# Vipermaseg/libagmv

Hardware: AMD Instinct MI355X
Metric: frames/s encode+decode (AGMV hot path: quantise+classify+assemble, parse+reconstruct), synthetic (higher is better)
Workload: dtype u8; 1 GPU; c3: 1024-frame 1920x1080 agmv_synth_v1, HIGH_QUALITY palette, OPT_III (512 colours); frames_per_gpu=1024, width=1920, height=1080, palette=512 colours, reference histogram build (GPU histogram + host pick), parallelism=1024 frames per rank, 1 rank(s), no data-path collective

## Files before the change

### libagmv_amd/csrc/agmv_decode_hip.hip

```cpp
#include <hip/hip_runtime.h>

#include <stdint.h>
#include <stdlib.h>
#include <string.h>
#include <type_traits>

#include "agmv_hip_impl.h"

#ifndef DEC_T_OVERRIDE
#define DEC_T_OVERRIDE 256
#endif
constexpr int DEC_T = DEC_T_OVERRIDE;
#ifndef DEC_BPB
#define DEC_BPB 24
#endif
constexpr int DEC_STAGE = DEC_T * DEC_BPB;
constexpr int DEC_SR = DEC_STAGE / 4 / DEC_T;
constexpr int DEC_MAX_SLICES = 32;

struct dec_ws {
	uint32_t* d_dirty;
	size_t dirty_cap;
	bool dep_split;
	uint32_t* d_parse_ws;
	size_t parse_ws_cap;
	uint32_t* d_fp_ws;
	size_t fp_ws_cap;
	uint32_t* d_fp_fstate;
	uint32_t fp_frames;
	uint32_t* d_fstate_call;
	size_t fstate_call_cap;
	uint32_t* d_nent_own;
	size_t nent_cap;
	hipStream_t aux_stream;
	hipEvent_t ev_fork;
	hipEvent_t ev_slice[DEC_MAX_SLICES];
};

static dec_ws* dec_area(agmv_hip_ctx* c) { return (dec_ws*)c->ws[AREA_DEC]; }

static void dec_free(void* p)
{
	dec_ws* d = (dec_ws*)p;
	(void)hipFree(d->d_dirty); (void)hipFree(d->d_parse_ws); (void)hipFree(d->d_fp_ws); (void)hipFree(d->d_nent_own);
	(void)hipFree(d->d_fstate_call);
	if (d->ev_fork) (void)hipEventDestroy(d->ev_fork);
	for (int i = 0; i < DEC_MAX_SLICES; i++) if (d->ev_slice[i]) (void)hipEventDestroy(d->ev_slice[i]);
	if (d->aux_stream) (void)hipStreamDestroy(d->aux_stream);
	free(d);
}

static int need_dec_ctx(agmv_hip_ctx* c, bool palette)
{
	if (agmv_hip_enter(c, palette)) return -1;
	return palette && !agmv_hip_area(c, AREA_DEC, sizeof(dec_ws), dec_free) ? -1 : 0;
}

template <class F>
static void dec_flags(F&& f) { f(); }
template <class F, class... Rest>
static void dec_flags(F&& f, bool flag, Rest... rest) { dec_flags([&](auto... r_) { if (flag) f(std::true_type(), r_...); else f(std::false_type(), r_...); }, rest...); }
#define DEC_LAUNCH(k, grid, block, s, A, ...) do { \
	dec_flags([&](auto... b_) { hipLaunchKernelGGL((k<decltype(b_)::value...>), grid, block, 0, s, A); }, __VA_ARGS__); \
	CK(hipGetLastError()); } while (0)

__device__ __forceinline__ bool is_flag(uint32_t b) { return b == FILL_FLAG || b == NORMAL_FLAG || b == COPY_FLAG; }

struct ByteSrc {
	const uint8_t* p;
	uint32_t cap;
	__device__ __forceinline__ uint32_t operator()(uint32_t pos) const { return pos < cap ? p[pos] : 0u; }
};

struct StagedSrc {
	const __attribute__((address_space(3))) uint8_t* lds;
	uint32_t lo, len;
	const uint8_t* p;
	uint32_t cap;
	__device__ __forceinline__ uint32_t operator()(uint32_t pos) const
	{
		const uint32_t d = pos - lo;
		if (d < len) return lds[d];
		return pos < cap ? p[pos] : 0u;
	}
};

__global__ __launch_bounds__(64) void k_parse_serial(const uint8_t* __restrict__ bits, unsigned long long stride,
                                                     const uint32_t* __restrict__ bpos_a, uint32_t n_frames,
                                                     uint32_t nblk, int mode512, uint32_t* __restrict__ offsets,
                                                     uint32_t* __restrict__ nentered)
// ... 81 lines not shown
struct ParseLds {
	uint8_t b[PC + PHALO];
	unsigned long long esc[PNSEG + 2];
	uint16_t jl[NLV][PC];
};

constexpr int PCD = ((PC + PHALO) / 4 + 63) / 64;

__device__ __forceinline__ void load_chunk(uint32_t (&raw)[PCD], const uint8_t* fbits, uint32_t cap, uint32_t cs, int lane)
{
#pragma unroll
	for (int q = 0; q < PCD; q++) {
		const uint32_t pos = cs + 4u * (uint32_t)(q * 64 + lane);
		raw[q] = (q * 64 + lane < (PC + PHALO) / 4 && pos < cap) ? *(const uint32_t*)(fbits + pos) : 0u;
	}
}

template <bool M512, int NLV>
__device__ __forceinline__ uint32_t parse_chunk_nodes(ParseLds<NLV>& S, uint16_t* rank_at, uint16_t* npos, uint16_t* eo, uint16_t* n0,
                                                      const uint32_t (&raw)[PCD], uint32_t bpos, uint32_t cs, int lane)
{
#pragma unroll
	for (int q = 0; q < PCD; q++) {
		const int i = q * 64 + lane;
		if (i < (PC + PHALO) / 4) ((uint32_t*)S.b)[i] = raw[q];
	}
	wave_lds_sync();
	uint32_t mtot = 0, by[PNSEG];
#pragma unroll
	for (int sg = 0; sg < PNSEG; sg++) by[sg] = S.b[sg * 64 + lane];
#pragma unroll
	for (int sg = 0; sg < PNSEG; sg++) {
		const uint32_t p = sg * 64 + lane;
		const bool node = is_flag(by[sg]) && cs + p <= bpos;
		const unsigned long long m = __ballot(node);
		const uint32_t r = mtot + __builtin_amdgcn_mbcnt_hi((uint32_t)(m >> 32), __builtin_amdgcn_mbcnt_lo((uint32_t)m, 0u));
		rank_at[p] = (uint16_t)r;
		if (node) npos[r] = (uint16_t)p;
		mtot += (uint32_t)__popcll(m);
		if (M512) {
			const unsigned long long em = __ballot((by[sg] & 0x7fu) == 127u);
			if (lane == 0) S.esc[sg] = em;
		}
	}
	if (M512) {
		const unsigned long long em = __ballot((S.b[PC + lane] & 0x7fu) == 127u);
		if (lane == 0) { S.esc[PNSEG] = em; S.esc[PNSEG + 1] = 0; }
	}
	wave_lds_sync();
	const bool more = cs + PC <= bpos;
	for (uint32_t k = lane; k < mtot; k += 64) {
		const uint32_t p = npos[k], byte = S.b[p];
		uint32_t e = p + 1u;
		if (byte == FILL_FLAG) e += M512 ? 1u + ((S.b[p + 1] & 0x7fu) == 127u ? 1u : 0u) : 1u;
		else if (byte == NORMAL_FLAG) {
			if (M512) {
				const uint32_t sg = e >> 6, sh = e & 63u;
				const unsigned long long lo = S.esc[sg], hi = S.esc[sg + 1];
				const uint32_t m = (uint32_t)(sh ? (lo >> sh) | (hi << (64u - sh)) : lo);
				uint32_t pos = 0;
#pragma unroll
				for (int i = 0; i < 16; i++) pos += 1u + ((m >> pos) & 1u);
				e += pos;
			} else e += 16u;
		}
		uint32_t j = J_END, n = 0;
		if (cs + e <= bpos) {
			n = 1;
			if (e >= (uint32_t)PC) j = J_EXIT | (e - PC);
			else {
				const uint32_t nx = rank_at[e];
				j = nx < mtot ? nx : (more ? J_EXIT : J_END);
			}
		}
		S.jl[0][k] = (uint16_t)j;
		if (eo) eo[k] = (uint16_t)(e | n << 15);
		if (n0) n0[k] = (uint16_t)n;
	}
	wave_lds_sync();
	return mtot;
}

template <bool M512>
__global__ __launch_bounds__(64) void k_parse_chunks(ParseArgs A)
{
	__shared__ ParseLds<2> S;
	__shared__ uint16_t nn[2][PC];
	const int lane = threadIdx.x;
	if (A.nbad && *A.nbad == 0) return;
	for (uint32_t f = blockIdx.y; f < A.n_frames; f += gridDim.y) {
	const uint32_t bpos = A.bpos[f], g0 = f * A.cpf, nch = parse_nch(A, f, bpos);
	const uint8_t* fbits = A.bits + (size_t)f * A.stride;
	uint32_t nxt[PCD];
	if (blockIdx.x < nch) load_chunk(nxt, fbits, (uint32_t)A.stride, blockIdx.x * PC, lane);
	for (uint32_t c = blockIdx.x; c < nch; c += gridDim.x) {
		const uint32_t g = g0 + c, cs = c * PC;
		uint32_t raw[PCD];
#pragma unroll
		for (int q = 0; q < PCD; q++) raw[q] = nxt[q];
		if (c + gridDim.x < nch) load_chunk(nxt, fbits, (uint32_t)A.stride, (c + gridDim.x) * PC, lane);
		if (A.vm && lane < PC / 64) A.vm[(size_t)f * A.maxR * FOWN + c * (PC / 64) + lane] = 0ull;
		const uint32_t mtot = parse_chunk_nodes<M512>(S,  nn[1],  S.jl[1], nullptr, nn[0], raw, bpos, cs, lane);
		const uint32_t k0 = lane < 33 ? nn[1][lane] : 0u;
		wave_lds_sync();
#pragma unroll
		for (int lv = 0; lv < PCL; lv++) {
			const uint16_t *js = S.jl[lv & 1], *ns = nn[lv & 1];
			uint16_t *jd = S.jl[(lv + 1) & 1], *nd = nn[(lv + 1) & 1];
			for (uint32_t k = lane; k < mtot; k += 64) {
				uint32_t j = js[k], n = ns[k];
				if (j < J_EXIT) { n += ns[j]; j = js[j]; }
				jd[k] = (uint16_t)j;
				nd[k] = (uint16_t)n;
			}
			wave_lds_sync();
		}
		if (lane < 33) {
			uint32_t ex = X_END, cnt = 0;
			if (cs + lane <= bpos) {
				uint32_t k = k0;
				if (k >= mtot) { if (cs + PC <= bpos) ex = 0; }
				else {
					const uint16_t *jf = S.jl[PCL & 1], *nf = nn[PCL & 1];
					do { cnt += nf[k]; k = jf[k]; } while (k < J_EXIT);
					if (k != J_END) ex = k & 0x3Fu;
				}
			}
			A.summ[(size_t)g * 33 + lane] = (uint16_t)(ex << 10 | cnt);
		}
		wave_lds_sync();
	}
	}
}

constexpr int PSB = 32;
__global__ __launch_bounds__(64) void k_parse_stitch(ParseArgs A)
{
	const int lane = threadIdx.x;
	if (A.nbad && *A.nbad == 0) return;
	for (uint32_t f = blockIdx.x; f < A.n_frames; f += gridDim.x) {
	const uint32_t c0 = f * A.cpf, nch = parse_nch(A, f, A.bpos[f]);
	if (nch == 0) continue;
	const uint16_t* rows = A.summ + (size_t)c0 * 33 + (lane < 33 ? lane : 0);
	uint32_t o = 0, kb = 0;
	uint32_t nxt[PSB];
#pragma unroll
	for (int u = 0; u < PSB; u++) nxt[u] = rows[(size_t)min((uint32_t)u, nch - 1u) * 33];
	for (uint32_t c = 0; c < nch; c += PSB) {
		uint32_t row[PSB];
#pragma unroll
		for (int u = 0; u < PSB; u++) row[u] = nxt[u];
#pragma unroll
		for (int u = 0; u < PSB; u++) nxt[u] = rows[(size_t)min(c + PSB + u, nch - 1u) * 33];
		uint32_t mine = 0;
#pragma unroll
		for (int u = 0; u < PSB; u++) {
			if (lane == u) mine = kb << 8 | o;
			if (c + u < nch && o != 0xFFu) {
				const uint32_t v = __builtin_amdgcn_readlane(row[u], __builtin_amdgcn_readfirstlane(o));
				kb += v & 0x3FFu;
				o = (v >> 10) == X_END ? 0xFFu : v >> 10;
			}
		}
		if (lane < PSB && c + lane < nch) A.centry[c0 + c + lane] = mine;
	}
	if (lane == 0) A.nentered[f] = min(A.nblk, kb + 1u);
	}
}

template <bool M512>
__global__ __launch_bounds__(64) void k_parse_emit(ParseArgs A)
{
	__shared__ ParseLds<PEL + 1> S;
	__shared__ uint16_t eo[PC];
	uint8_t* mark = S.b;
	static_assert(PEL >= 2 && PC + PHALO >= PC, "rank_at / npos borrow jl[PEL-1] / jl[PEL], the marks borrow the bytes");
	const int lane = threadIdx.x;
	if (A.nbad && *A.nbad == 0) return;
	for (uint32_t f = blockIdx.y; f < A.n_frames; f += gridDim.y) {
	const uint32_t bpos = A.bpos[f], g0 = f * A.cpf, nch = parse_nch(A, f, bpos);
	const uint8_t* fbits = A.bits + (size_t)f * A.stride;
	uint32_t* off = A.offsets + (size_t)f * A.nblk;
	uint32_t nxt[PCD], ce_n = 0;
	if (blockIdx.x < nch) { ce_n = A.centry[g0 + blockIdx.x]; load_chunk(nxt, fbits, (uint32_t)A.stride, blockIdx.x * PC, lane); }
	for (uint32_t c = blockIdx.x; c < nch; c += gridDim.x) {
		const uint32_t ce = ce_n, o = ce & 0xFFu, kb = ce >> 8;
		uint32_t raw[PCD];
#pragma unroll
		for (int q = 0; q < PCD; q++) raw[q] = nxt[q];
		if (c + gridDim.x < nch) {
			ce_n = A.centry[g0 + c + gridDim.x];
			load_chunk(nxt, fbits, (uint32_t)A.stride, (c + gridDim.x) * PC, lane);
		}
		unsigned long long* fvm = A.vm ? A.vm + (size_t)f * A.maxR * FOWN : nullptr;
		if (c == 0 && lane == 0) {
			if (fvm) atomicOr(fvm, 1ull); else off[0] = 0;
		}
		if (o == 0xFFu) continue;
		if (kb + 1u >= A.nblk) continue;
		const uint32_t cs = c * PC;
		const uint32_t mtot = parse_chunk_nodes<M512>(S,  S.jl[PEL - 1],  S.jl[PEL], eo, nullptr, raw, bpos, cs, lane);
		const uint32_t k0 = cs + o <= bpos ? S.jl[PEL - 1][o] : mtot;
		for (uint32_t k = lane; k < mtot; k += 64) mark[k] = 0;
		wave_lds_sync();
		if (k0 < mtot) {
#pragma unroll
			for (int lv = 0; lv < PEL; lv++) {
				for (uint32_t k = lane; k < mtot; k += 64) {
					uint32_t j = S.jl[lv][k];
					if (j < J_EXIT) j = S.jl[lv][j];
					S.jl[lv + 1][k] = (uint16_t)j;
				}
				wave_lds_sync();
			}
			if (lane == 0)
				for (uint32_t k = k0; k < J_EXIT; k = S.jl[PEL][k]) mark[k] = 1;
			wave_lds_sync();
#pragma unroll
			for (int lv = PEL - 1; lv >= 0; lv--) {
				for (uint32_t k = lane; k < mtot; k += 64) {
					const uint32_t j = S.jl[lv][k];
					if (mark[k] && j < J_EXIT) mark[j] = 1;
				}
				wave_lds_sync();
			}
			uint32_t base = kb + 1u;
			for (uint32_t kg = 0; kg < mtot; kg += 64) {
				const uint32_t k = kg + lane;
				const uint32_t ev = k < mtot ? eo[k] : 0u;
				const bool on = k < mtot && mark[k] && (ev & 0x8000u);
				const unsigned long long m = __ballot(on);
				const uint32_t kk = base + __builtin_amdgcn_mbcnt_hi((uint32_t)(m >> 32), __builtin_amdgcn_mbcnt_lo((uint32_t)m, 0u));
				if (on && kk < A.nblk) {
					const uint32_t pos = cs + (ev & 0x7FFFu);
					if (fvm) atomicOr(fvm + (pos >> 6), 1ull << (pos & 63u)); else off[kk] = pos;
				}
				base += (uint32_t)__popcll(m);
			}
		}
		wave_lds_sync();
	}
	}
}

constexpr int FROW = FC / 4 + 1;
constexpr uint32_t FX_SLIDE = 64u, FX_END = 65u, FX_UNSET = 66u, FX_MERGE = 128u;
constexpr int FP_REPAIRS = 24;
constexpr int FP_LDS = 64 * FROW + 1;

struct FpArgs {
	const uint8_t* bits;
	unsigned long long stride;
	const uint32_t* bpos;
	uint4* rec;
	unsigned long long* vm;
	uint32_t* kb;
	uint32_t* fstate;
	uint32_t* offsets;
	uint32_t* nentered;
	uint32_t n_frames, nblk, maxR;
	uint32_t* nbad;
	uint32_t* tidx;
	uint32_t tpfd;
	uint32_t* dirty;
	uint32_t ndirty;
};
constexpr uint32_t TIDX_NONE = 0xFFFFFFFFu;

__device__ __forceinline__ __amdgpu_buffer_rsrc_t uniform_rsrc(const void* p, uint32_t bytes)
{
	const uint64_t a = (uint64_t)p;
	const uint32_t lo = (uint32_t)__builtin_amdgcn_readfirstlane((int)(uint32_t)a), hi = (uint32_t)__builtin_amdgcn_readfirstlane((int)(uint32_t)(a >> 32));
	return __builtin_amdgcn_make_buffer_rsrc((void*)((uint64_t)hi << 32 | lo), 0, __builtin_amdgcn_readfirstlane((int)bytes), 0x00020000);
}

__device__ __forceinline__ uint32_t ctz64(unsigned long long m) { return (uint32_t)__builtin_ctzll(m); }
__device__ __forceinline__ unsigned long long above(uint32_t q) { return (~0ull << q) << 1; }

template <bool M512>
__device__ __forceinline__ void fp_walk_region(const FpArgs& A, uint32_t* s_b, uint32_t f, uint32_t r, uint32_t forced, uint32_t bpos, int lane)
{
	const uint8_t* fbits = A.bits + (size_t)f * A.stride;
	const uint32_t cap = (uint32_t)A.stride;
	const long sb = (long)r * FRB - FH * FC;
	uint32_t raw[16];
	{
		const __amdgpu_buffer_rsrc_t rs = uniform_rsrc(fbits, cap & ~3u);
		const uint32_t o0 = (sb < 0 ? 0xFFFFFF00u : (uint32_t)sb) + 4u * (uint32_t)lane;
		const uint32_t o1 = (uint32_t)(sb + FH * FC) + 4u * (uint32_t)lane;
		raw[0] = (uint32_t)__builtin_amdgcn_raw_buffer_load_b32(rs, o0, 0, 0);
#pragma unroll
		for (int k = 1; k < 16; k++) raw[k] = (uint32_t)__builtin_amdgcn_raw_buffer_load_b32(rs, o1 + 256u * (uint32_t)(k - 1), 0, 0);
	}
	{
		uint32_t* row = s_b + (lane >> 4) * FROW + (lane & 15);
#pragma unroll
		for (int k = 0; k < 16; k++) row[k * 4 * FROW] = raw[k];
	}
	wave_lds_sync();
	const long cb = sb + (long)lane * FC;
	unsigned long long F, C, L, E = 0;
	{
		auto zero7 = [](uint32_t v) -> uint32_t { return ~(((v & 0x7F7F7F7Fu) + 0x7F7F7F7Fu) | v) & 0x80808080u; };
		uint32_t f2[2] = {0, 0}, c2[2] = {0, 0}, lc2[2] = {0, 0}, e2[2] = {0, 0};
		auto place = [](uint32_t acc, uint32_t x128, int sh) -> uint32_t { return acc | (sh == 0 ? x128 >> 7 : x128 << (sh - 7)); };
		auto pair128 = [](uint32_t z0, uint32_t z1) -> uint32_t {
			return __builtin_amdgcn_udot4(z1, 0x80402010u, __builtin_amdgcn_udot4(z0, 0x08040201u, 0u, false), false);
		};
#pragma unroll
		for (int j = 0; j < 16; j += 2) {
			const uint32_t w0 = s_b[lane * FROW + j], w1 = s_b[lane * FROW + j + 1];
			const uint32_t zlc0 = zero7((w0 | 0x10101010u) ^ 0x5E5E5E5Eu), zn0 = zero7(w0 ^ 0x2F2F2F2Fu);
			const uint32_t zlc1 = zero7((w1 | 0x10101010u) ^ 0x5E5E5E5Eu), zn1 = zero7(w1 ^ 0x2F2F2F2Fu);
			const int h = j >> 3, sh = 4 * (j & 7);
			lc2[h] = place(lc2[h], pair128(zlc0, zlc1), sh);
			c2[h] = place(c2[h], pair128(zlc0 & (w0 << 3), zlc1 & (w1 << 3)), sh);
			f2[h] = place(f2[h], pair128(zlc0 | zn0, zlc1 | zn1), sh);
			if (M512) e2[h] = place(e2[h], pair128(((w0 & 0x7F7F7F7Fu) + 0x01010101u) & 0x80808080u, ((w1 & 0x7F7F7F7Fu) + 0x01010101u) & 0x80808080u), sh);
		}
		F = (unsigned long long)f2[1] << 32 | f2[0]; C = (unsigned long long)c2[1] << 32 | c2[0];
		L = ((unsigned long long)lc2[1] << 32 | lc2[0]) ^ C; E = (unsigned long long)e2[1] << 32 | e2[0];
	}
	const long lim_l = (long)bpos - cb;
	const int lim = lim_l > 1000 ? 1000 : (lim_l < -1000 ? -1000 : (int)lim_l);
// ... 2 lines not shown
		const long nv = lim_l + 1;
		const unsigned long long ok = nv <= 0 ? 0ull : (nv < 64 ? (1ull << nv) - 1ull : ~0ull);
		F &= ok;
		safe = ok >> 3;
	}
	const bool more = lim >= FC;
	unsigned long long En = 0;
	unsigned long long D;
	{
		unsigned long long L3 = 0;
		if (M512) {
			const uint32_t lo = (uint32_t)__shfl_down((int)(uint32_t)E, 1, 64), hi = (uint32_t)__shfl_down((int)(uint32_t)(E >> 32), 1, 64);
			En = lane < 63 ? ((unsigned long long)hi << 32 | lo) : 0ull;
			L3 = L & ((E >> 1) | (En << 63));
			L &= ~L3;
		}
		D = (F & ~(C | L | L3)) | (F & ((L << 1) | (L3 << 1) | (L3 << 2))) | (F & ~safe);
	}
	const int first = forced != FX_UNSET ? FH : 0;
	const bool walker = lane >= first && lane < 63 && cb >= 0;
	const uint32_t* mine = s_b + lane * FROW;
	const uint32_t behind = mine[FROW];
	unsigned long long V = 0, Q = 0;
	uint32_t xo = FX_UNSET, applied = FX_UNSET;
	uint32_t want = (lane == first && forced != FX_UNSET) ? forced : FX_SLIDE;
	for (int round = 0; round < 66; round++) {
		const bool need = walker && want != applied;
		if (__ballot(need) == 0) break;
		bool go = false;
		uint32_t q = 0, res = xo;
		unsigned long long Vw = 0, Qw = 0;
		if (need) {
			applied = want;
			if (want == FX_END) { V = 0; Q = 0; res = FX_END; }
			else {
				const uint32_t x = want == FX_SLIDE ? 0u : want;
				Vw = want == FX_SLIDE ? 0ull : 1ull << x;
				const unsigned long long m = F >> x;
				if (m == 0) { V = Vw; Q = 0; res = more ? FX_SLIDE : FX_END; }
				else {
					q = x + ctz64(m);
					if ((Q >> q) & 1ull) { V = Vw | (V & above(q)); Q &= ~0ull << q; }
					else go = true;
				}
			}
		}
		uint32_t wres = FX_UNSET;
		for (;;) {
			if (__ballot(go) == 0) break;
			{
				const bool merged = go && ((Q >> q) & 1ull);
				wres = merged ? FX_MERGE + q : wres;
				go = go && !merged;
			}
			const unsigned long long hiq = ~0ull << q;
			const unsigned long long dq = (D & hiq) | (Q & (hiq << 1));
			const uint32_t d = dq ? ctz64(dq) : 64u;
			const bool str = go && d != q;
			if (__ballot(str) != 0) {
				const unsigned long long nodes = F & hiq & (d >= 64u ? ~0ull : ~(~0ull << d));
				const uint32_t last = 63u - (uint32_t)__builtin_clzll(nodes | 1ull);
				const uint32_t e = last + (((C >> last) & 1ull) ? 1u : (((L >> last) & 1ull) ? 2u : 3u));
				Qw |= str ? nodes : 0ull;
				Vw |= str ? ((nodes & C) << 1) | ((nodes & L) << 2) | ((nodes & ~(C | L)) << 3) : 0ull;
				const unsigned long long m = F >> (e & 63u);
				const bool inside = e < 64u && m != 0;
				const uint32_t stop = e >= 64u ? e - 64u : (more ? FX_SLIDE : FX_END);
				wres = (str && !inside) ? stop : wres;
				const uint32_t p = e + ctz64(m | (1ull << 63));
				const bool arrived = str && inside;
				const bool merged = arrived && ((Q >> (p & 63u)) & 1ull);
				wres = merged ? FX_MERGE + p : wres;
				q = arrived ? p : q;
				go = go && (!str || (inside && !merged));
			}
			const bool sing = go && ((D >> q) & 1ull);
			if (__ballot(sing) != 0) {
				const uint32_t d0 = mine[q >> 2], d1 = mine[(q >> 2) + 1];
				const uint32_t two = __builtin_amdgcn_alignbyte((q >> 2) == 15u ? behind : d1, d0, q & 3u);
				const uint32_t t = two & 0xFFu;
				const bool isN = t == NORMAL_FLAG, isC = t == COPY_FLAG;
				uint32_t l1 = isC ? 1u : 2u + ((M512 && ((two >> 8) & 0x7Fu) == 127u) ? 1u : 0u);
				if (__ballot(sing && isN) != 0) {
					uint32_t len = 16;
					if (M512) {
						const uint32_t q1 = q + 1u;
						const uint32_t m = (uint32_t)((q1 < 64u ? E >> q1 : 0ull) | (En << (63u - q)));
						uint32_t pos = 0;
#pragma unroll
						for (int i = 0; i < 16; i++) pos += 1u + ((m >> pos) & 1u);
						len = pos;
					}
					if (isN) l1 = 1u + len;
				}
				const uint32_t e = q + l1;
				const bool over = (int)e > lim;
				const bool cnt = sing && !over;
				Qw |= cnt ? 1ull << q : 0ull;
				Vw |= cnt ? (1ull << q) << l1 : 0ull;
				const unsigned long long m = F >> (e & 63u);
				const bool inside = cnt && e < 64u && m != 0;
				const uint32_t stop = over ? FX_END : (e >= 64u ? e - 64u : (more ? FX_SLIDE : FX_END));
				wres = (sing && !inside) ? stop : wres;
				q = inside ? e + ctz64(m) : q;
				go = go && (!sing || inside);
			}
		}
		if (need && wres != FX_UNSET) {
			if (wres >= FX_MERGE) {
				const uint32_t mq = wres - FX_MERGE;
				V = Vw | (V & above(mq)); Q = Qw | (Q & (~0ull << mq));
			} else { V = Vw; Q = Qw; res = wres; }
		}
		if (need) xo = res;
		const uint32_t px = (uint32_t)__shfl_up((int)xo, 1, 64);
		if (walker && lane > first) want = px;
	}
	const bool own = lane >= FH && lane < 63;
	if (own) A.vm[((size_t)f * A.maxR + r) * FOWN + (lane - FH)] = walker ? V : 0ull;
	const uint32_t n = wave_sum(own && walker ? (uint32_t)__popcll(V) : 0u);
	const uint32_t ein = forced != FX_UNSET ? forced : (uint32_t)__builtin_amdgcn_readlane((int)xo, FH - 1);
	const uint32_t xout = (uint32_t)__builtin_amdgcn_readlane((int)xo, 62);
	if (lane == 0) A.rec[(size_t)f * A.maxR + r] = make_uint4(ein, xout, n, 0u);
	wave_lds_sync();
}

template <bool M512>
__global__ __launch_bounds__(64) __attribute__((amdgpu_waves_per_eu(6, 8))) void k_fp_walk(FpArgs A)
{
	__shared__ uint32_t s_b[FP_LDS];
	const int lane = threadIdx.x;
	if (blockIdx.x == 0 && blockIdx.y == 0 && lane == 0) *A.nbad = 0;
	for (uint32_t f = blockIdx.y; f < A.n_frames; f += gridDim.y) {
		const uint32_t bpos = A.bpos[f];
		const uint32_t nreg = min(bpos / FRB + 1u, A.maxR);
		for (uint32_t r = blockIdx.x; r < nreg; r += gridDim.x)
			fp_walk_region<M512>(A, s_b, f, r, r == 0 ? 0u : FX_UNSET, bpos, lane);
	}
}

template <bool M512>
__global__ __launch_bounds__(64) __attribute__((amdgpu_waves_per_eu(8, 8))) void k_fp_finish(FpArgs A)
{
	__shared__ uint32_t s_b[FP_LDS];
	const uint32_t f = blockIdx.x;
	const int lane = threadIdx.x;
	const uint32_t bpos = A.bpos[f];
	const uint32_t nreg = min(bpos / FRB + 1u, A.maxR);
	uint4* rec = A.rec + (size_t)f * A.maxR;
	if (A.tidx)
		for (uint32_t t = lane; t <= A.tpfd; t += 64) A.tidx[(size_t)f * (A.tpfd + 1) + t] = TIDX_NONE;
	int budget = FP_REPAIRS;
	for (uint32_t start = 1;;) {
		uint32_t bad = 0xFFFFFFFFu;
		for (uint32_t r0 = start & ~63u; r0 < nreg && bad == 0xFFFFFFFFu; r0 += 64) {
			const uint32_t r = r0 + lane;
			const bool in = r < nreg && r >= start;
			const uint32_t x = in ? __hip_atomic_load(&rec[r].x, __ATOMIC_RELAXED, __HIP_MEMORY_SCOPE_AGENT) : 0u;
			const uint32_t yp = in ? __hip_atomic_load(&rec[r - 1].y, __ATOMIC_RELAXED, __HIP_MEMORY_SCOPE_AGENT) : 0u;
			const unsigned long long bm = __ballot(in && x != yp);
			if (bm) bad = r0 + ctz64(bm);
		}
		if (bad == 0xFFFFFFFFu) break;
		if (budget-- == 0) {
			if (lane == 0) { A.fstate[f] = FS_BAD; atomicAdd(A.nbad, 1u); }
			return;
		}
		const uint32_t want = __builtin_amdgcn_readfirstlane(__hip_atomic_load(&rec[bad - 1].y, __ATOMIC_RELAXED, __HIP_MEMORY_SCOPE_AGENT));
		fp_walk_region<M512>(A, s_b, f, bad, want, bpos, lane);
		__builtin_amdgcn_fence(__ATOMIC_RELEASE, "agent");
		__builtin_amdgcn_fence(__ATOMIC_ACQUIRE, "agent");
		start = bad + 1;
	}
	uint32_t run = 0;
	for (uint32_t r0 = 0; r0 < nreg; r0 += 64) {
		const uint32_t r = r0 + lane;
// ... 602 lines not shown
	else {
#pragma unroll
		for (int k = 0; k < 16; k++) cur[k] = 0;
	}
	if (A.prev_iframe) load_block(A.prev_iframe, poff, A.w, icol);
	else {
#pragma unroll
		for (int k = 0; k < 16; k++) icol[k] = 0;
	}
	uint32_t stale = 0xFFFFu, istale = 0xFFFFu;
	bool dep = false;
	for (uint32_t f = 0; f < A.n_frames; f++) {
		bool fill_written = false;
		const uint32_t own3 = cur[3], own3s = (stale >> 3) & 1u;
		if (active && blk < A.nentered[f]) {
			ByteSrc src{A.bits + (size_t)f * A.stride, (uint32_t)A.stride};
			const uint32_t o = BM ? bm_offset_of(A.vm, A.kb, A.maxR, A.bpos[f], f, blk) : A.offsets[(size_t)f * A.nblk + blk];
			decode_block<M512>(src, o, A.bpos[f], s_pal, cur, icol, istale, stale, fill_written);
		}
		const int nbl = nb_lane < 0 ? 0 : nb_lane;
		const uint32_t left = (uint32_t)__builtin_amdgcn_readlane((int)cur[7], nbl);
		const uint32_t lefts = ((uint32_t)__builtin_amdgcn_readlane((int)stale, nbl) >> 7) & 1u;
		if (is_last && fill_written) {
			const uint32_t c = A.bw == 1 ? own3 : left;
#pragma unroll
			for (int k = 0; k < 16; k++) cur[k] = c;
			stale = (A.bw == 1 ? own3s : lefts) ? 0xFFFFu : 0u;
		}
		if (((A.first_fc + f) & 3u) == 0) {
#pragma unroll
			for (int k = 0; k < 16; k++) icol[k] = cur[k];
			istale = stale;
		}
		if (active) store_block(A.out + (size_t)f * npx, poff, A.w, cur);
		if (active && stale) dep = true;
	}
	if (dep) A.dirty[nwords + 1] = 1u;
}

static int check_slab(const uint8_t* d_bits, size_t stride)
{
	if ((stride & 3u) || stride < 4 || ((uintptr_t)d_bits & 3u)) return agmv_hip_err("agmv_hip: bitstream slab and stride must be 4-byte aligned");
	return 0;
}

struct DecRows {
	const uint8_t* bits;
	size_t stride;
	const uint32_t* bpos;
	uint32_t *offsets, *nentered;
	uint32_t n_frames, nblk;
};
static DecRows rows_range(DecRows r, uint32_t f0, uint32_t f1)
{
	r.bits += (size_t)f0 * r.stride; r.bpos += f0; r.nentered += f0; r.n_frames = f1 - f0;
	if (r.offsets) r.offsets += (size_t)f0 * r.nblk;
	return r;
}
struct DecPix {
	uint32_t w, h, first_fc;
	uint32_t* out;
	const uint32_t *prev, *prev_iframe;
};

static uint32_t dirty_words(uint32_t nblk) { return (nblk + 31) / 32 + 2; }

enum ParseMode { PARSE_FAST, PARSE_ROBUST, PARSE_SERIAL };
static ParseMode parse_mode()
{
	const char* m = getenv("AGMV_HIP_PARSE");
	return !m ? PARSE_FAST : strcmp(m, "robust") == 0 ? PARSE_ROBUST : strcmp(m, "serial") == 0 ? PARSE_SERIAL : PARSE_FAST;
}

static uint32_t parse_grid_x(agmv_hip_ctx* c, uint32_t n_frames, size_t cap)
{
	uint32_t gx = (uint32_t)(((size_t)c->n_cu * 512 + n_frames - 1) / n_frames);
	if (gx < 32) gx = 32;
	if (gx > 256) gx = 256;
	if (gx > cap) gx = (uint32_t)cap;
	return gx < 1 ? 1 : gx;
}

static int parse_launch_robust(agmv_hip_ctx* c, const DecRows& r, size_t ws_frames, hipStream_t s,
                               const uint32_t* fstate, const uint32_t* nbad, unsigned long long* vm, uint32_t maxR)
{
	const size_t cpf = (r.stride + PC) / PC, maxchunks = cpf * ws_frames;
	if (maxchunks >> 32) return agmv_hip_err("agmv_hip: parser batch too large (%zu chunk rows)", maxchunks);
	dec_ws* d = dec_area(c);
	CK(agmv_hip_dev_grow(&d->d_parse_ws, &d->parse_ws_cap, (maxchunks + (maxchunks * 33 + 1) / 2 + 16) * 4, 1));
	ParseArgs A;
	memset(&A, 0, sizeof(A));
	A.bits = r.bits; A.stride = r.stride; A.bpos = r.bpos; A.offsets = r.offsets; A.nentered = r.nentered;
	A.cpf = (uint32_t)cpf; A.centry = d->d_parse_ws; A.summ = (uint16_t*)(A.centry + maxchunks);
	A.n_frames = r.n_frames; A.nblk = r.nblk; A.fstate = fstate; A.vm = vm; A.maxR = maxR; A.nbad = nbad;
	const uint32_t n = r.n_frames;
	const dim3 grid(parse_grid_x(c, n, fstate && cpf > 32 ? 32 : cpf), fstate ? (n < 64u ? n : 64u) : (n < 65535u ? n : 65535u));
	const int m512 = c->mode512;
	DEC_LAUNCH(k_parse_chunks, grid, dim3(64), s, A, m512);
	hipLaunchKernelGGL(k_parse_stitch, dim3(fstate ? (n < 1024u ? n : 1024u) : n), dim3(64), 0, s, A);
	CK(hipGetLastError());
	DEC_LAUNCH(k_parse_emit, grid, dim3(64), s, A, m512);
	return 0;
}

static int parse_launch(agmv_hip_ctx* c, const DecRows& r, size_t ws_frames, hipStream_t s, DecArgs* bm, uint32_t* fstate = nullptr)
{
	const bool robust_only = parse_mode() == PARSE_ROBUST;
	const uint32_t n_frames = r.n_frames;
	dec_ws* d = dec_area(c);
	d->d_fp_fstate = nullptr; d->fp_frames = 0;
	if (!bm && (n_frames > 65535u || robust_only)) return parse_launch_robust(c, r, ws_frames, s, nullptr, nullptr, nullptr, 0);
	if (n_frames > 65535u) return agmv_hip_err("agmv_hip: more than 65535 frames in one parser launch");
	const size_t maxR = (r.stride + FRB - 1) / FRB + 1, nreg = maxR * ws_frames;
	const uint32_t tpfd = (r.nblk + DEC_T - 1) / DEC_T;
	const size_t b_rec = nreg * sizeof(uint4), b_vm = nreg * FOWN * 8, b_kb = nreg * 4, b_fs = ((ws_frames * 4 + 15) & ~(size_t)15);
	const size_t b_tx = bm ? (((size_t)ws_frames * (tpfd + 1) * 4 + 15) & ~(size_t)15) : 0;
	CK(agmv_hip_dev_grow(&d->d_fp_ws, &d->fp_ws_cap, b_rec + b_vm + b_kb + b_fs + b_tx + 16, 1));
	FpArgs A;
	memset(&A, 0, sizeof(A));
	A.bits = r.bits; A.stride = r.stride; A.bpos = r.bpos; A.offsets = r.offsets; A.nentered = r.nentered;
	uint8_t* w = (uint8_t*)d->d_fp_ws;
	A.rec = (uint4*)w; A.vm = (unsigned long long*)(w + b_rec); A.kb = (uint32_t*)(w + b_rec + b_vm); A.fstate = (uint32_t*)(w + b_rec + b_vm + b_kb);
	if (fstate) A.fstate = fstate;
	A.tidx = bm ? (uint32_t*)(w + b_rec + b_vm + b_kb + b_fs) : nullptr; A.tpfd = tpfd;
	A.nbad = (uint32_t*)(w + b_rec + b_vm + b_kb + b_fs + b_tx);
	A.n_frames = n_frames; A.nblk = r.nblk; A.maxR = (uint32_t)maxR;
	if (bm) { A.dirty = bm->dirty; A.ndirty = dirty_words(r.nblk); }
	uint32_t gx = parse_grid_x(c, n_frames, maxR);
	uint32_t gy = n_frames;
	if ((size_t)gx * gy > 131072u) {
		const uint32_t want = (uint32_t)(((size_t)r.stride / 8 + FRB - 1) / FRB) + 1;
		if (gx > want) gx = want;
		if ((size_t)gx * gy > 131072u) gy = 131072u / gx;
	} else if (bm) {
		const size_t worst = (size_t)r.nblk * (c->mode512 ? 33 : 17) + 64;
		const uint32_t want = (uint32_t)((worst / 8 + FRB - 1) / FRB) + 1;
		if (gx > want && (size_t)want * gy >= (size_t)c->n_cu * 32 * 4) gx = want;
	}
	const dim3 grid(gx, gy);
	if (robust_only) {
		CK(hipMemsetAsync(A.tidx, 0xFF, (size_t)n_frames * (tpfd + 1) * 4, s));
		CK(hipMemsetAsync(A.vm, 0, (size_t)n_frames * maxR * FOWN * 8, s));
		CK(hipMemsetD32Async((hipDeviceptr_t)A.fstate, (int)FS_BAD, n_frames, s));
		CK(hipMemsetD32Async((hipDeviceptr_t)A.nbad, (int)n_frames, 1, s));
	} else {
		DEC_LAUNCH(k_fp_walk, grid, dim3(64), s, A, c->mode512);
		DEC_LAUNCH(k_fp_finish, dim3(n_frames), dim3(64), s, A, c->mode512);
	}
	d->d_fp_fstate = A.fstate; d->fp_frames = n_frames;
	if (!bm) {
		hipLaunchKernelGGL(k_fp_expand, dim3(gx, n_frames), dim3(64), 0, s, A);
		CK(hipGetLastError());
		return parse_launch_robust(c, r, ws_frames, s, A.fstate, A.nbad, nullptr, 0);
	}
	bm->vm = A.vm; bm->kb = A.kb; bm->tidx = A.tidx; bm->maxR = A.maxR;
	if (parse_launch_robust(c, r, ws_frames, s, A.fstate, A.nbad, A.vm, A.maxR)) return -1;
	hipLaunchKernelGGL(k_fp_tiles, dim3(gx / 2 ? gx / 2 : 1, gy), dim3(64), 0, s, A);
	CK(hipGetLastError());
	return 0;
}

extern "C" int agmv_hip_parse_frames_dev(agmv_hip_ctx* c, const uint8_t* d_bits, size_t stride, const uint32_t* d_bpos,
                                         uint32_t n_frames, uint32_t w, uint32_t h, uint32_t* d_offsets, uint32_t* d_nentered,
                                         void* stream)
{
	if (need_dec_ctx(c, true)) return -1;
	if (agmv_hip_check_geometry(w, h)) return -1;
	if (n_frames == 0) return 0;
	const DecRows r = {d_bits, stride, d_bpos, d_offsets, d_nentered, n_frames, (w / 4) * (h / 4)};
	hipStream_t s = (hipStream_t)stream;
	if (parse_mode() == PARSE_SERIAL) {
		hipLaunchKernelGGL(k_parse_serial, dim3((n_frames + 63) / 64), dim3(64), 0, s, d_bits,
		                   (unsigned long long)stride, d_bpos, n_frames, r.nblk, c->mode512, d_offsets, d_nentered);
		CK(hipGetLastError());
		return 0;
	}
	if (check_slab(d_bits, stride)) return -1;
	agmv_hip_ev_mark(c, 2, s);
	if (parse_launch(c, r, n_frames, s, nullptr)) return -1;
	agmv_hip_ev_mark(c, 3, s);
	return 0;
}

extern "C" int agmv_hip_parse_fallback_frames(agmv_hip_ctx* c, void* stream)
{
	if (need_dec_ctx(c, false)) return -1;
	const dec_ws* d = dec_area(c);
	if (!d || !d->d_fp_fstate || d->fp_frames == 0) return 0;
	CK(hipStreamSynchronize((hipStream_t)stream));
	uint32_t* h = (uint32_t*)malloc((size_t)d->fp_frames * 4);
	if (!h) return agmv_hip_err("agmv_hip: out of host memory");
	if (hipMemcpy(h, d->d_fp_fstate, (size_t)d->fp_frames * 4, hipMemcpyDeviceToHost) != hipSuccess) { free(h); agmv_hip_err("agmv_hip: D2H failed"); return -1; }
	int n = 0;
	for (uint32_t i = 0; i < d->fp_frames; i++) n += h[i] != FS_OK;
	free(h);
	return n;
}

static int decode_prepare(agmv_hip_ctx* c, DecArgs& A, const DecRows& r, const DecPix& px, hipStream_t s, bool clear, bool second = false)
{
	if (((uintptr_t)px.out & 15u) || ((uintptr_t)px.prev & 15u) || ((uintptr_t)px.prev_iframe & 15u)) return agmv_hip_err("agmv_hip: pixel buffers must be 16-byte aligned");
	if (check_slab(r.bits, r.stride)) return -1;
	memset(&A, 0, sizeof(A));
	A.bits = r.bits; A.stride = r.stride; A.bpos = r.bpos; A.offsets = r.offsets; A.nentered = r.nentered;
	A.out = px.out; A.pal = c->d_pal; A.prev = px.prev; A.prev_iframe = px.prev_iframe;
	A.n_frames = r.n_frames; A.w = px.w; A.h = px.h; A.bw = px.w / 4; A.nblk = r.nblk;
	A.tpf = (A.nblk + DEC_T - 1) / DEC_T;
	A.first_fc = px.first_fc; A.phase = px.first_fc & 3u; A.n_groups = (r.n_frames + A.phase + 3) / 4;
	const size_t nwords = dirty_words(A.nblk);
	dec_ws* d = dec_area(c);
	CK(agmv_hip_dev_grow(&d->d_dirty, &d->dirty_cap, 2 * nwords * 4, 1));
	A.dirty = d->d_dirty + (second ? nwords : 0); d->dep_split = false;
	if (clear) CK(hipMemsetAsync(A.dirty, 0, nwords * 4, s));
	return 0;
}

static int decode_launch(agmv_hip_ctx* c, DecArgs A, uint32_t g0, uint32_t g1, hipStream_t s)
{
	A.grp0 = g0; A.n_items = (g1 - g0) * A.tpf;
	uint32_t nwg = A.n_items;
	if (const char* e = getenv("AGMV_DEC_GRID")) {
		const long n = atol(e);
		if (n > 0 && (unsigned long)n < nwg) nwg = (uint32_t)n;
	}
	DEC_LAUNCH(k_decode, dim3(nwg), dim3(DEC_T), s, A, c->mode512, A.vm != nullptr, nwg < A.n_items);
	return 0;
}

static int fixup_launch(agmv_hip_ctx* c, const DecArgs& A, hipStream_t s)
{
	DEC_LAUNCH(k_fixup, dim3((A.nblk + 63) / 64), dim3(64), s, A, c->mode512, A.vm != nullptr);
	return 0;
}

extern "C" int agmv_hip_decode_frames_dev(agmv_hip_ctx* c, const uint8_t* d_bits, size_t stride, const uint32_t* d_bpos,
                                          const uint32_t* d_offsets, const uint32_t* d_nentered, uint32_t n_frames,
                                          uint32_t w, uint32_t h, uint32_t first_fc, uint32_t* d_out,
                                          const uint32_t* d_prev, const uint32_t* d_prev_iframe, void* stream)
{
// ... 173 lines not shown
```

Before: 222,800 frames/s.

## Fuse robust parser fallback into one launch and speed normal-block length scan

When the fast parser path has run, the three robust-parser kernels (chunks, stitch, emit) are replaced by a single kernel. It runs only on frames marked bad, using four waves per block that share LDS through a union, with block barriers between stages. This removes two kernel launches and full-grid passes over frames that mostly need no fallback. Separately, the 16-step bit-walk that computes a normal block's length in 512-colour mode is replaced with an 8-step lookup using byte-permute on 3-bit windows, which shortens the serial dependency chain in the walk kernel. The fused fallback handles each bad frame with only four waves, so many bad frames could run slower.

```diff
diff --git a/libagmv_amd/csrc/agmv_decode_hip.hip b/libagmv_amd/csrc/agmv_decode_hip.hip
--- a/libagmv_amd/csrc/agmv_decode_hip.hip
+++ b/libagmv_amd/csrc/agmv_decode_hip.hip
@@ -6,6 +6,7 @@
 #include <type_traits>
 
 #include "agmv_hip_impl.h"
+#include "agmv_fp_len.h"
 
 #ifndef DEC_T_OVERRIDE
 #define DEC_T_OVERRIDE 256
@@ -253,23 +254,18 @@
 }
 
 template <bool M512>
-__global__ __launch_bounds__(64) void k_parse_chunks(ParseArgs A)
-{
-	__shared__ ParseLds<2> S;
-	__shared__ uint16_t nn[2][PC];
-	const int lane = threadIdx.x;
-	if (A.nbad && *A.nbad == 0) return;
-	for (uint32_t f = blockIdx.y; f < A.n_frames; f += gridDim.y) {
+__device__ __forceinline__ void parse_chunks_frame(const ParseArgs& A, ParseLds<2>& S, uint16_t (&nn)[2][PC], uint32_t f, uint32_t cfirst, uint32_t cstep, int lane)
+{
 	const uint32_t bpos = A.bpos[f], g0 = f * A.cpf, nch = parse_nch(A, f, bpos);
 	const uint8_t* fbits = A.bits + (size_t)f * A.stride;
 	uint32_t nxt[PCD];
-	if (blockIdx.x < nch) load_chunk(nxt, fbits, (uint32_t)A.stride, blockIdx.x * PC, lane);
-	for (uint32_t c = blockIdx.x; c < nch; c += gridDim.x) {
+	if (cfirst < nch) load_chunk(nxt, fbits, (uint32_t)A.stride, cfirst * PC, lane);
+	for (uint32_t c = cfirst; c < nch; c += cstep) {
 		const uint32_t g = g0 + c, cs = c * PC;
 		uint32_t raw[PCD];
 #pragma unroll
 		for (int q = 0; q < PCD; q++) raw[q] = nxt[q];
-		if (c + gridDim.x < nch) load_chunk(nxt, fbits, (uint32_t)A.stride, (c + gridDim.x) * PC, lane);
+		if (c + cstep < nch) load_chunk(nxt, fbits, (uint32_t)A.stride, (c + cstep) * PC, lane);
 		if (A.vm && lane < PC / 64) A.vm[(size_t)f * A.maxR * FOWN + c * (PC / 64) + lane] = 0ull;
 		const uint32_t mtot = parse_chunk_nodes<M512>(S,  nn[1],  S.jl[1], nullptr, nn[0], raw, bpos, cs, lane);
 		const uint32_t k0 = lane < 33 ? nn[1][lane] : 0u;
@@ -301,17 +297,23 @@
 		}
 		wave_lds_sync();
 	}
-	}
-}
-
-constexpr int PSB = 32;
-__global__ __launch_bounds__(64) void k_parse_stitch(ParseArgs A)
-{
+}
+
+template <bool M512>
+__global__ __launch_bounds__(64) void k_parse_chunks(ParseArgs A)
+{
+	__shared__ ParseLds<2> S;
+	__shared__ uint16_t nn[2][PC];
 	const int lane = threadIdx.x;
 	if (A.nbad && *A.nbad == 0) return;
-	for (uint32_t f = blockIdx.x; f < A.n_frames; f += gridDim.x) {
+	for (uint32_t f = blockIdx.y; f < A.n_frames; f += gridDim.y) parse_chunks_frame<M512>(A, S, nn, f, blockIdx.x, gridDim.x, lane);
+}
+
+constexpr int PSB = 32;
+__device__ __forceinline__ void parse_stitch_frame(const ParseArgs& A, uint32_t f, int lane)
+{
 	const uint32_t c0 = f * A.cpf, nch = parse_nch(A, f, A.bpos[f]);
-	if (nch == 0) continue;
+	if (nch == 0) return;
 	const uint16_t* rows = A.summ + (size_t)c0 * 33 + (lane < 33 ? lane : 0);
 	uint32_t o = 0, kb = 0;
 	uint32_t nxt[PSB];
@@ -336,32 +338,33 @@
 		if (lane < PSB && c + lane < nch) A.centry[c0 + c + lane] = mine;
 	}
 	if (lane == 0) A.nentered[f] = min(A.nblk, kb + 1u);
-	}
+}
+
+__global__ __launch_bounds__(64) void k_parse_stitch(ParseArgs A)
+{
+	const int lane = threadIdx.x;
+	if (A.nbad && *A.nbad == 0) return;
+	for (uint32_t f = blockIdx.x; f < A.n_frames; f += gridDim.x) parse_stitch_frame(A, f, lane);
 }
 
 template <bool M512>
-__global__ __launch_bounds__(64) void k_parse_emit(ParseArgs A)
-{
-	__shared__ ParseLds<PEL + 1> S;
-	__shared__ uint16_t eo[PC];
+__device__ __forceinline__ void parse_emit_frame(const ParseArgs& A, ParseLds<PEL + 1>& S, uint16_t (&eo)[PC], uint32_t f, uint32_t cfirst, uint32_t cstep, int lane)
+{
 	uint8_t* mark = S.b;
 	static_assert(PEL >= 2 && PC + PHALO >= PC, "rank_at / npos borrow jl[PEL-1] / jl[PEL], the marks borrow the bytes");
-	const int lane = threadIdx.x;
-	if (A.nbad && *A.nbad == 0) return;
-	for (uint32_t f = blockIdx.y; f < A.n_frames; f += gridDim.y) {
 	const uint32_t bpos = A.bpos[f], g0 = f * A.cpf, nch = parse_nch(A, f, bpos);
 	const uint8_t* fbits = A.bits + (size_t)f * A.stride;
 	uint32_t* off = A.offsets + (size_t)f * A.nblk;
 	uint32_t nxt[PCD], ce_n = 0;
-	if (blockIdx.x < nch) { ce_n = A.centry[g0 + blockIdx.x]; load_chunk(nxt, fbits, (uint32_t)A.stride, blockIdx.x * PC, lane); }
-	for (uint32_t c = blockIdx.x; c < nch; c += gridDim.x) {
+	if (cfirst < nch) { ce_n = A.centry[g0 + cfirst]; load_chunk(nxt, fbits, (uint32_t)A.stride, cfirst * PC, lane); }
+	for (uint32_t c = cfirst; c < nch; c += cstep) {
 		const uint32_t ce = ce_n, o = ce & 0xFFu, kb = ce >> 8;
 		uint32_t raw[PCD];
 #pragma unroll
 		for (int q = 0; q < PCD; q++) raw[q] = nxt[q];
-		if (c + gridDim.x < nch) {
-			ce_n = A.centry[g0 + c + gridDim.x];
-			load_chunk(nxt, fbits, (uint32_t)A.stride, (c + gridDim.x) * PC, lane);
+		if (c + cstep < nch) {
+			ce_n = A.centry[g0 + c + cstep];
+			load_chunk(nxt, fbits, (uint32_t)A.stride, (c + cstep) * PC, lane);
 		}
 		unsigned long long* fvm = A.vm ? A.vm + (size_t)f * A.maxR * FOWN : nullptr;
 		if (c == 0 && lane == 0) {
@@ -411,6 +414,37 @@
 		}
 		wave_lds_sync();
 	}
+}
+
+template <bool M512>
+__global__ __launch_bounds__(64) void k_parse_emit(ParseArgs A)
+{
+	__shared__ ParseLds<PEL + 1> S;
+	__shared__ uint16_t eo[PC];
+	const int lane = threadIdx.x;
+	if (A.nbad && *A.nbad == 0) return;
+	for (uint32_t f = blockIdx.y; f < A.n_frames; f += gridDim.y) parse_emit_frame<M512>(A, S, eo, f, blockIdx.x, gridDim.x, lane);
+}
+
+constexpr int PFW = 4;
+template <bool M512>
+__global__ __launch_bounds__(64 * PFW) void k_parse_fallback(ParseArgs A)
+{
+	struct Stage1 { ParseLds<2> S; uint16_t nn[2][PC]; };
+	struct Stage3 { ParseLds<PEL + 1> S; uint16_t eo[PC]; };
+	union WaveLds { Stage1 a; Stage3 b; };
+	__shared__ WaveLds L[PFW];
+	if (*A.nbad == 0) return;
+	const int lane = threadIdx.x & 63;
+	const uint32_t w = threadIdx.x >> 6;
+	for (uint32_t f = blockIdx.x; f < A.n_frames; f += gridDim.x) {
+		if (A.fstate[f] != FS_BAD) continue;
+		parse_chunks_frame<M512>(A, L[w].a.S, L[w].a.nn, f, w, PFW, lane);
+		__syncthreads();
+		if (w == 0) parse_stitch_frame(A, f, lane);
+		__syncthreads();
+		parse_emit_frame<M512>(A, L[w].b.S, L[w].b.eo, f, w, PFW, lane);
+		__syncthreads();
 	}
 }
 
@@ -579,16 +613,13 @@
 				const bool isN = t == NORMAL_FLAG, isC = t == COPY_FLAG;
 				uint32_t l1 = isC ? 1u : 2u + ((M512 && ((two >> 8) & 0x7Fu) == 127u) ? 1u : 0u);
 				if (__ballot(sing && isN) != 0) {
-					uint32_t len = 16;
+					uint32_t sz = 17;
 					if (M512) {
-						const uint32_t q1 = q + 1u;
-						const uint32_t m = (uint32_t)((q1 < 64u ? E >> q1 : 0ull) | (En << (63u - q)));
-						uint32_t pos = 0;
-#pragma unroll
-						for (int i = 0; i < 16; i++) pos += 1u + ((m >> pos) & 1u);
-						len = pos;
+						const bool up = q >= 32u;
+						const uint32_t lo = up ? (uint32_t)(E >> 32) : (uint32_t)E, hi = up ? (uint32_t)En : (uint32_t)(E >> 32);
+						sz = fp_normal_size8(__builtin_amdgcn_alignbit(hi, lo, q));
 					}
-					if (isN) l1 = 1u + len;
+					if (isN) l1 = sz;
 				}
 				const uint32_t e = q + l1;
 				const bool over = (int)e > lim;
@@ -1357,7 +1388,7 @@
 }
 
 static int parse_launch_robust(agmv_hip_ctx* c, const DecRows& r, size_t ws_frames, hipStream_t s,
-                               const uint32_t* fstate, const uint32_t* nbad, unsigned long long* vm, uint32_t maxR)
+                               const uint32_t* fstate, const uint32_t* nbad, unsigned long long* vm, uint32_t maxR, bool one_launch = false)
 {
 	const size_t cpf = (r.stride + PC) / PC, maxchunks = cpf * ws_frames;
 	if (maxchunks >> 32) return agmv_hip_err("agmv_hip: parser batch too large (%zu chunk rows)", maxchunks);
@@ -1369,8 +1400,12 @@
 	A.cpf = (uint32_t)cpf; A.centry = d->d_parse_ws; A.summ = (uint16_t*)(A.centry + maxchunks);
 	A.n_frames = r.n_frames; A.nblk = r.nblk; A.fstate = fstate; A.vm = vm; A.maxR = maxR; A.nbad = nbad;
 	const uint32_t n = r.n_frames;
+	const int m512 = c->mode512;
+	if (one_launch) {
+		DEC_LAUNCH(k_parse_fallback, dim3(n < 256u ? n : 256u), dim3(64 * PFW), s, A, m512);
+		return 0;
+	}
 	const dim3 grid(parse_grid_x(c, n, fstate && cpf > 32 ? 32 : cpf), fstate ? (n < 64u ? n : 64u) : (n < 65535u ? n : 65535u));
-	const int m512 = c->mode512;
 	DEC_LAUNCH(k_parse_chunks, grid, dim3(64), s, A, m512);
 	hipLaunchKernelGGL(k_parse_stitch, dim3(fstate ? (n < 1024u ? n : 1024u) : n), dim3(64), 0, s, A);
 	CK(hipGetLastError());
@@ -1426,10 +1461,10 @@
 	if (!bm) {
 		hipLaunchKernelGGL(k_fp_expand, dim3(gx, n_frames), dim3(64), 0, s, A);
 		CK(hipGetLastError());
-		return parse_launch_robust(c, r, ws_frames, s, A.fstate, A.nbad, nullptr, 0);
+		return parse_launch_robust(c, r, ws_frames, s, A.fstate, A.nbad, nullptr, 0, true);
 	}
 	bm->vm = A.vm; bm->kb = A.kb; bm->tidx = A.tidx; bm->maxR = A.maxR;
-	if (parse_launch_robust(c, r, ws_frames, s, A.fstate, A.nbad, A.vm, A.maxR)) return -1;
+	if (parse_launch_robust(c, r, ws_frames, s, A.fstate, A.nbad, A.vm, A.maxR, !robust_only)) return -1;
 	hipLaunchKernelGGL(k_fp_tiles, dim3(gx / 2 ? gx / 2 : 1, gy), dim3(64), 0, s, A);
 	CK(hipGetLastError());
 	return 0;
diff --git a/libagmv_amd/csrc/agmv_fp_len.h b/libagmv_amd/csrc/agmv_fp_len.h
--- /dev/null
+++ b/libagmv_amd/csrc/agmv_fp_len.h
@@ -0,0 +1,33 @@
+#ifndef AGMV_FP_LEN_H
+#define AGMV_FP_LEN_H
+#include <stdint.h>
+
+#if defined(__HIPCC__) || defined(__CUDACC__)
+#define AGMV_HD __host__ __device__ __forceinline__
+#else
+#define AGMV_HD static inline
+#endif
+
+AGMV_HD uint32_t fp_normal_len16(uint32_t m)
+{
+	uint32_t pos = 0;
+	for (int i = 0; i < 16; i++) pos += 1u + ((m >> pos) & 1u);
+	return pos;
+}
+
+constexpr uint32_t FP_LEN2_LO = 0x03030302u, FP_LEN2_HI = 0x04030402u;
+AGMV_HD uint32_t fp_normal_size8(uint32_t m1)
+{
+	uint32_t pos = 1;
+#if defined(__HIP_DEVICE_COMPILE__)
+#pragma unroll
+	for (int i = 0; i < 8; i++) pos += __builtin_amdgcn_perm(FP_LEN2_HI, FP_LEN2_LO, __builtin_amdgcn_ubfe(m1, pos, 3u));
+	return pos & 0xFFu;
+#else
+	const uint64_t tab = (uint64_t)FP_LEN2_HI << 32 | FP_LEN2_LO;
+	for (int i = 0; i < 8; i++) pos += (uint32_t)(tab >> (8u * ((m1 >> pos) & 7u))) & 0xFFu;
+	return pos;
+#endif
+}
+
+#endif
```

New measurement: 223,500 frames/s, median of 6. About the same (+0.3%).
